# 3DHumanRehab/MOSS

Measured on AMD Instinct MI355X. Metric: train iters/sec (fwd+bwd, 512x512, ~100k Gaussians), higher is better.
Workload: dtype f32; 1 GPU; BASELINE configs[2]: 100000 Gaussians on a synthetic capsule body, 512x512, SH degree 3, step = render + L1 + 0.2(1-SSIM) + 0.5 maskL2 + backward + AdamW; one view per GPU per step; MOSS's data flow (scales + rotations + a per-Gaussian LBS transform per frame, gaussian_renderer/__init__.py:88-93) with the covariance product, the getters, the loss and AdamW as this library's kernels and the step re; target=body, input_mode=lbs, index_order=as_generated, activations=in_op, P=100000, visible=100000, num_rendered=240441, pixels=262144, parallelism=single GPU, forward=async, launch=one hipGraph replay per step, loss=full frame: L1 + 0.2 (1 - SSIM) + 0.5 mask L2 (moss_photometric_loss)

## Files before the change

moss_amd/csrc/preprocess.hip:

```cpp
#include "common.h"
#include "adamw.h"

namespace moss {

namespace {

struct M3 { float m[3][3]; };

__device__ __forceinline__ float sigmoid_act(float v) { return 1.0f / (1.0f + expf(-v)); }
__device__ __forceinline__ void activate_scale_rot(int raw, float* sc, float* q)
{
    if (raw & RAW_SCALE) { sc[0] = expf(sc[0]); sc[1] = expf(sc[1]); sc[2] = expf(sc[2]); }
    if (raw & RAW_ROTATION) {
        const float n = sqrtf(q[0] * q[0] + q[1] * q[1] + q[2] * q[2] + q[3] * q[3]);
        const float inv = 1.0f / fmaxf(n, 1e-12f);
        q[0] *= inv; q[1] *= inv; q[2] *= inv; q[3] *= inv;
    }
}
__device__ __forceinline__ void normalize_backward(const float* q, const float* y, float* g)
{
    const float n = sqrtf(q[0] * q[0] + q[1] * q[1] + q[2] * q[2] + q[3] * q[3]);
    const float inv = 1.0f / fmaxf(n, 1e-12f);
    const float yg = n >= 1e-12f ? (y[0] * g[0] + y[1] * g[1] + y[2] * g[2] + y[3] * g[3]) : 0.0f;
#pragma unroll
// ... 520 lines not shown
    for (int k = 0; k < 3; k++) dmean[k] = Rv[0][k] * dt[0] + Rv[1][k] * dt[1] + Rv[2][k] * dt[2];

    {
        const float hx = projmatrix[0] * mean.x + projmatrix[4] * mean.y + projmatrix[8] * mean.z + projmatrix[12];
        const float hy = projmatrix[1] * mean.x + projmatrix[5] * mean.y + projmatrix[9] * mean.z + projmatrix[13];
        const float hw = projmatrix[3] * mean.x + projmatrix[7] * mean.y + projmatrix[11] * mean.z + projmatrix[15];
        const float iw = 1.0f / (hw + 0.0000001f);
        const float nx = hx * iw, ny = hy * iw;
#pragma unroll
        for (int k = 0; k < 3; k++)
            dmean[k] += iw * ((projmatrix[4 * k] - nx * projmatrix[4 * k + 3]) * gmx + (projmatrix[4 * k + 1] - ny * projmatrix[4 * k + 3]) * gmy);
    }

}

__device__ __forceinline__ void scale_rot_backward(int idx, const float* dcov, const float (&A)[2][3], const float (&d2)[3],
                                                   float scale_modifier, int raw,
                                                   bool has_scales, const float (&sc_in)[3], const float (&q_in)[4],
                                                   bool has_transforms, const float (&Tm)[9], float* dscale, float* drot, float* dtf)
{
    (void)idx;
    if (has_scales) {
        float scr[3] = { sc_in[0], sc_in[1], sc_in[2] };
        float qr[4] = { q_in[0], q_in[1], q_in[2], q_in[3] };
        const float q_raw[4] = { qr[0], qr[1], qr[2], qr[3] };
        activate_scale_rot(raw, scr, qr);
        float Ap[2][3] = { { A[0][0], A[0][1], A[0][2] }, { A[1][0], A[1][1], A[1][2] } };
        float d6[6] = { dcov[0], dcov[1], dcov[2], dcov[3], dcov[4], dcov[5] };
        if (has_transforms) {
            float pre[6], d6_pre[6];
            cov3d_from_scale_rot(scr, scale_modifier, qr, pre);
            transform_cov3d_bw(Tm, pre, d6, d6_pre, dtf);
#pragma unroll
            for (int i = 0; i < 6; i++) d6[i] = d6_pre[i];
#pragma unroll
            for (int j = 0; j < 2; j++)
#pragma unroll
                for (int i = 0; i < 3; i++) Ap[j][i] = A[j][0] * Tm[i] + A[j][1] * Tm[3 + i] + A[j][2] * Tm[6 + i];
        }
        const float qw = qr[0], qx = qr[1], qy = qr[2], qz = qr[3];
        const float R[3][3] = { { 1.f - 2.f * (qy * qy + qz * qz), 2.f * (qx * qy - qw * qz), 2.f * (qx * qz + qw * qy) },
                                { 2.f * (qx * qy + qw * qz), 1.f - 2.f * (qx * qx + qz * qz), 2.f * (qy * qz - qw * qx) },
                                { 2.f * (qx * qz - qw * qy), 2.f * (qy * qz + qw * qx), 1.f - 2.f * (qx * qx + qy * qy) } };
        const float sm[3] = { scale_modifier * scr[0], scale_modifier * scr[1], scale_modifier * scr[2] };
        const float D3[3][3] = { { d6[0], 0.5f * d6[1], 0.5f * d6[2] }, { 0.5f * d6[1], d6[3], 0.5f * d6[4] }, { 0.5f * d6[2], 0.5f * d6[4], d6[5] } };
        float G[3][3];
#pragma unroll
        for (int k = 0; k < 3; k++) {
            const float u0 = Ap[0][0] * R[0][k] + Ap[0][1] * R[1][k] + Ap[0][2] * R[2][k];
            const float u1 = Ap[1][0] * R[0][k] + Ap[1][1] * R[1][k] + Ap[1][2] * R[2][k];
            const float w0 = d2[0] * u0 + d2[1] * u1, w1 = d2[1] * u0 + d2[2] * u1;
            dscale[k] = 2.0f * sm[k] * (u0 * w0 + u1 * w1);
            float col[3];
#pragma unroll
            for (int i = 0; i < 3; i++) col[i] = 2.0f * sm[k] * (D3[i][0] * R[0][k] + D3[i][1] * R[1][k] + D3[i][2] * R[2][k]);
#pragma unroll
            for (int i = 0; i < 3; i++) G[i][k] = col[i] * sm[k];
        }
        const float a0 = G[2][1] - G[1][2], a1 = G[0][2] - G[2][0], a2q = G[1][0] - G[0][1];
        const float s01 = G[0][1] + G[1][0], s02 = G[0][2] + G[2][0], s12 = G[1][2] + G[2][1];
        const float trG = G[0][0] + G[1][1] + G[2][2];
        drot[0] = 2.0f * (qx * a0 + qy * a1 + qz * a2q);
        drot[1] = 2.0f * (qy * s01 + qz * s02 + qw * a0) - 4.0f * qx * (trG - G[0][0]);
        drot[2] = 2.0f * (qx * s01 + qz * s12 + qw * a1) - 4.0f * qy * (trG - G[1][1]);
        drot[3] = 2.0f * (qx * s02 + qy * s12 + qw * a2q) - 4.0f * qz * (trG - G[2][2]);
        if (raw & RAW_SCALE) {
#pragma unroll
            for (int k = 0; k < 3; k++) dscale[k] *= scr[k];
        }
        if (raw & RAW_ROTATION) normalize_backward(q_raw, qr, drot);
    }
}

__device__ __forceinline__ uint32_t run_word_mask(uint32_t word, uint32_t c0, uint32_t c1)
{
    const uint32_t base = word << 5;
    const uint32_t lo = c0 > base ? c0 - base : 0u, hi = c1 > base ? min(c1 - base, 32u) : 0u;
    if (hi <= lo) return 0u;
    return (hi >= 32u ? 0xffffffffu : ((1u << hi) - 1u)) & ~((1u << lo) - 1u);
}
template <int NG>
__device__ __forceinline__ void coop_gather(bool is_big, uint32_t c0, uint32_t c1,
                                            const uint32_t* __restrict__ cell_valid, const float4* __restrict__ inst_grad, float* sums)
    {
        typedef float v4f __attribute__((ext_vector_type(4)));
        constexpr uint32_t OOB = 0xffffffffu, RSRC3 = 0x00020000u;
        constexpr uint32_t LPR = 64u / (uint32_t)NG;
        const __amdgpu_buffer_rsrc_t rs_msk = __builtin_amdgcn_make_buffer_rsrc((void*)cell_valid, 0, 0xffffff00u, RSRC3);
        const __amdgpu_buffer_rsrc_t rs_rec = __builtin_amdgcn_make_buffer_rsrc((void*)inst_grad, 0, 0xffffff00u, RSRC3);
        unsigned long long big = __ballot(is_big);
        const uint32_t lane = threadIdx.x & 63u, grp = lane / LPR, j = lane % LPR;
        while (big) {
            int src[NG];
#pragma unroll
            for (int g = 0; g < NG; g++) { src[g] = big ? __ffsll(big) - 1 : -1; big &= big - 1ull; }
            int my_src = src[0];
#pragma unroll
            for (int g = 1; g < NG; g++) my_src = grp == (uint32_t)g ? src[g] : my_src;
            const uint32_t bc0 = __shfl(c0, max(my_src, 0)), bc1_any = __shfl(c1, max(my_src, 0));
            const uint32_t bc1 = my_src >= 0 ? bc1_any : bc0;
            uint32_t nmax = 0u;
#pragma unroll
            for (int g = 0; g < NG; g++) {
                const uint32_t n = src[g] >= 0 ? (uint32_t)__builtin_amdgcn_readlane((int)(c1 - c0), max(src[g], 0)) : 0u;
                nmax = max(nmax, n);
            }
            float acc[9] = { 0, 0, 0, 0, 0, 0, 0, 0, 0 };
            constexpr int CPL = 8;
            for (uint32_t r0 = 0u; r0 < nmax; r0 += LPR * CPL) {
                uint32_t vw[CPL];
#pragma unroll
                for (int i = 0; i < CPL; i++) {
                    const uint32_t cell = bc0 + r0 + LPR * (uint32_t)i + j;
                    vw[i] = __builtin_amdgcn_raw_buffer_load_b32(rs_msk, cell < bc1 ? (cell >> 5) * 4u : OOB, 0, 0);
                }
                v4f ra[CPL], rb[CPL]; float rc[CPL];
#pragma unroll
                for (int i = 0; i < CPL; i++) {
                    const uint32_t cell = bc0 + r0 + LPR * (uint32_t)i + j;
                    const bool on = ((vw[i] >> (cell & 31u)) & 1u) != 0u;
                    const uint32_t o = on ? cell * (uint32_t)(GRAD_REC_FLOATS * 4) : OOB;
                    ra[i] = __builtin_amdgcn_raw_buffer_load_b128(rs_rec, o, 0, 0);
                    rb[i] = __builtin_amdgcn_raw_buffer_load_b128(rs_rec, on ? o + 16u : OOB, 0, 0);
                    rc[i] = __builtin_bit_cast(float, __builtin_amdgcn_raw_buffer_load_b32(rs_rec, on ? o + 32u : OOB, 0, 0));
                }
#pragma unroll
                for (int i = 0; i < CPL; i++) {
                    acc[0] += ra[i].x; acc[1] += ra[i].y; acc[2] += ra[i].z; acc[3] += ra[i].w;
                    acc[4] += rb[i].x; acc[5] += rb[i].y; acc[6] += rb[i].z; acc[7] += rb[i].w;
                    acc[8] += rc[i];
                }
            }
#pragma unroll
            for (int q = 0; q < 9; q++) {
#pragma unroll
                for (int d = (int)LPR / 2; d >= 1; d >>= 1) acc[q] += __shfl_xor(acc[q], d);
            }
#pragma unroll
            for (int g = 0; g < NG; g++) {
                if (src[g] >= 0) {
#pragma unroll
                    for (int q = 0; q < 9; q++) {
                        const float v = __builtin_bit_cast(float, __builtin_amdgcn_readlane(__builtin_bit_cast(int, acc[q]), g * (int)LPR));
                        if ((int)lane == src[g]) sums[q] = v;
                    }
                }
            }
        }
    }

constexpr int SH_ROW = 49;
constexpr int GATHER_CAP = 320;
constexpr int GATHER_WORDS = GATHER_CAP + 64 * 9;
template <bool STAGE_SH, bool FUSED, int LPG_L2 >
__global__ void __launch_bounds__(256) __attribute__((amdgpu_waves_per_eu(2)))
preprocess_backward_kernel(int P, int D, int M, float tan_fovx, float tan_fovy, float h_x, float h_y, float mean2d_sx, float mean2d_sy,
                           float scale_modifier,
                           const float* __restrict__ means3D, const float* __restrict__ shs,
                           const float* __restrict__ scales, const float* __restrict__ rotations,
                           const float* __restrict__ cov3D_precomp, const float* __restrict__ viewmatrix,
                           const float* __restrict__ projmatrix, const float* __restrict__ cam_pos,
                           GeomView g, const float4* __restrict__ inst_grad ,
                           const uint32_t* __restrict__ cell_valid , const uint32_t* __restrict__ header,
                           float* __restrict__ dL_dmean2D, float* __restrict__ dL_dconic, float* __restrict__ dL_dopacity,
                           float* __restrict__ dL_dcolor, float* __restrict__ dL_dmean3D, float* __restrict__ dL_dcov3D,
                           float* __restrict__ dL_dsh, float* __restrict__ dL_dscale, float* __restrict__ dL_drot,
                           const float* __restrict__ transforms, float* __restrict__ dL_dtransforms,
                           const float* __restrict__ opacities , int raw,
                           unsigned long long* __restrict__ g_stamps_dev ,
                           uint32_t* __restrict__ queues,
                           const float* __restrict__ translation , float* __restrict__ dL_dtranslation ,
                           FusedAdam fa )
{
    if (queues != nullptr && blockIdx.x == 0 && threadIdx.x < 2 * NUM_XCD_QUEUES) {
        const int line = threadIdx.x < NUM_XCD_QUEUES ? Q_BWD + (int)threadIdx.x : Q_SEG_HEAD + (int)threadIdx.x - NUM_XCD_QUEUES;
        queues[(size_t)line * QLINE_WORDS] = 0u;
    }
    float fa_bc1 = 1.0f, fa_bc2_sqrt = 1.0f;
    int fa_t = 0;
    extern __shared__ float s_sh[];
#define PSTAMP(i) if (g_stamps_dev && threadIdx.x == 0) g_stamps_dev[(size_t)blockIdx.x * 16 + (i)] = __builtin_amdgcn_s_memtime()
#define PRSTAMP(i) if (g_stamps_dev && threadIdx.x == 0) g_stamps_dev[(size_t)blockIdx.x * 16 + (i)] = __builtin_amdgcn_s_memrealtime()
    PSTAMP(0); PRSTAMP(13);
    float* const s_dsh = s_sh;
    const int gl2 = (raw >> 12) & 7;
#define rows_used ((int)blockDim.x >> LPG_L2)
    constexpr int lpg_l2 = LPG_L2;
    auto gaussian_of_row = [&](int r) -> int {
        if constexpr (LPG_L2 == 0) { return (((r >> gl2) * (int)gridDim.x + (int)blockIdx.x) << gl2) + (r & ((1 << gl2) - 1)); }
        else { return (r & ((1 << LPG_L2) - 1)) ? 0x7fffffff : (int)blockIdx.x * rows_used + (r >> LPG_L2); }
    };
    const int idx = gaussian_of_row((int)threadIdx.x);
    const bool in_range = idx < P;
    const int idc = min(idx, P - 1);
    constexpr int SH_J = LPG_L2 == 0 ? 12 : 1;
    typedef float v4f_sh __attribute__((ext_vector_type(4)));
    constexpr uint32_t SH_OOB = 0xffffffffu;
    const int na_D = (3 * (D + 1) * (D + 1) + 3) >> 2;
    const __amdgpu_buffer_rsrc_t rs_shs = __builtin_amdgcn_make_buffer_rsrc((void*)shs, 0, 0xffffff00u, 0x00020000u);
    v4f_sh shv[12];
    if (STAGE_SH) {
        const size_t total4 = (size_t)P * 12;
#pragma unroll
        for (int j = 0; j < SH_J; j++) {
            const int f = (int)threadIdx.x + j * (int)blockDim.x;
            size_t a;
            if constexpr (LPG_L2 == 0) a = min((size_t)gaussian_of_row(f / 12) * 12 + (size_t)(f % 12), total4 - 1);
            else a = f / 12 < rows_used ? min((size_t)min(gaussian_of_row((f / 12) << lpg_l2), P - 1) * 12 + (size_t)(f % 12), total4 - 1) : total4 - 1;
            shv[j] = __builtin_amdgcn_raw_buffer_load_b128(rs_shs, (f % 12) < na_D ? (uint32_t)a * 16u : SH_OOB, 0, 0);
        }
    }
    const uint32_t tt_raw = g.tiles_touched[idc], off_raw = g.rec_offsets[idc] + g.group_rbase[idc >> 8], cells_raw = g.rec_count[idc], hdr_flags = header[2];
    float in_x[3], in_T[9] = { 0.f, 0.f, 0.f, 0.f, 0.f, 0.f, 0.f, 0.f, 0.f }, in_t[3] = { 0.f, 0.f, 0.f }, in_c6[6], in_sc[3] = { 0.f, 0.f, 0.f }, in_q[4] = { 0.f, 0.f, 0.f, 0.f };
    float in_opa = 0.f;
#pragma unroll
    for (int i = 0; i < 3; i++) in_x[i] = means3D[3 * (size_t)idc + i];
    if (transforms != nullptr) {
#pragma unroll
        for (int i = 0; i < 9; i++) in_T[i] = transforms[9 * (size_t)idc + i];
    }
    if ((raw & RAW_POSE) && translation != nullptr) {
#pragma unroll
        for (int i = 0; i < 3; i++) in_t[i] = translation[3 * (size_t)idc + i];
    }
    {
        const float* c6p = (cov3D_precomp != nullptr) ? cov3D_precomp + 6 * (size_t)idc : g.cov3D + 6 * (size_t)idc;
#pragma unroll
        for (int i = 0; i < 6; i++) in_c6[i] = c6p[i];
    }
    if (scales != nullptr) {
#pragma unroll
        for (int i = 0; i < 3; i++) in_sc[i] = scales[3 * (size_t)idc + i];
#pragma unroll
        for (int i = 0; i < 4; i++) in_q[i] = rotations[4 * (size_t)idc + i];
    }
    if (raw & RAW_OPACITY) in_opa = opacities[idc];
    const uint8_t in_clamped = g.clamped[idc];
    if (STAGE_SH) {
#pragma unroll
        for (int j = 0; j < SH_J; j++) {
            const int f = threadIdx.x + j * blockDim.x;
            if (LPG_L2 == 0 || f / 12 < rows_used) {
                float* d = &s_sh[((f / 12) << lpg_l2) * SH_ROW + (f % 12) * 4];
                d[0] = shv[j].x; d[1] = shv[j].y; d[2] = shv[j].z; d[3] = shv[j].w;
            }
        }
    }
    const uint32_t n_inst = in_range ? tt_raw : 0u;
#pragma unroll
    for (int i = 0; i < 3; i++) { asm volatile("" : "+v"(in_x[i])); asm volatile("" : "+v"(in_t[i])); asm volatile("" : "+v"(in_sc[i])); }
#pragma unroll
    for (int i = 0; i < 9; i++) asm volatile("" : "+v"(in_T[i]));
#pragma unroll
    for (int i = 0; i < 6; i++) asm volatile("" : "+v"(in_c6[i]));
#pragma unroll
    for (int i = 0; i < 4; i++) asm volatile("" : "+v"(in_q[i]));
    asm volatile("" : "+v"(in_opa));
    float3 gcol = make_float3(0, 0, 0); float gmx = 0, gmy = 0, gca = 0, gcb = 0, gcc = 0, gop = 0;
    float dmean[3] = { 0, 0, 0 }, dcov[6] = { 0, 0, 0, 0, 0, 0 }, dscale[3] = { 0, 0, 0 }, drot[4] = { 0, 0, 0, 0 };
    float dtf[9] = { 0, 0, 0, 0, 0, 0, 0, 0, 0 }, dpose_t[3] = { 0, 0, 0 };
    float A_cov[2][3] = { { 0, 0, 0 }, { 0, 0, 0 } }, d2_cov[3] = { 0, 0, 0 };
    const bool visible = n_inst > 0 && !(hdr_flags & (ERRFLAG_OVERFLOW | ERRFLAG_FORWARD_ONLY));
    const bool fa_on = FUSED && !(hdr_flags & (ERRFLAG_OVERFLOW | ERRFLAG_FORWARD_ONLY));

    constexpr uint32_t COOP_WORDS = 16, MID_CELLS = 96;
    const uint32_t c0 = visible ? off_raw : 0u, c1 = c0 + (visible ? cells_raw : 0u);
    const uint32_t word0 = c0 >> 5, n_words = c1 > c0 ? ((c1 + 31u) >> 5) - word0 : 0u;
    const bool mid_size = LPG_L2 == 0 && (c1 - c0) > MID_CELLS && n_words <= COOP_WORDS;
    {
        const bool mine = n_words != 0u && n_words <= COOP_WORDS && !mid_size;
        PSTAMP(8);
        const int lane_g = (int)(threadIdx.x & 63u);
        uint32_t g_c0 = c0, g_c1 = c1, g_n = mine ? n_words : 0u;
        if constexpr (LPG_L2 == 4) {
            g_c0 = (uint32_t)__shfl((int)g_c0, lane_g & ~15); g_c1 = (uint32_t)__shfl((int)g_c1, lane_g & ~15); g_n = (uint32_t)__shfl((int)g_n, lane_g & ~15);
        }
        const bool has_word = (uint32_t)(lane_g & 15) < g_n;
        uint32_t wmax = LPG_L2 == 4 ? (has_word ? 1u : 0u) : (mine ? n_words : 0u);
#pragma unroll
        for (int d = 32; d >= 1; d >>= 1) wmax = max(wmax, (uint32_t)__shfl_xor((int)wmax, d));
        typedef float v4f __attribute__((ext_vector_type(4)));
        constexpr uint32_t OOB = 0xffffffffu, RSRC3 = 0x00020000u;
        const __amdgpu_buffer_rsrc_t rs_msk = __builtin_amdgcn_make_buffer_rsrc((void*)cell_valid, 0, 0xffffff00u, RSRC3);
        const __amdgpu_buffer_rsrc_t rs_rec = __builtin_amdgcn_make_buffer_rsrc((void*)inst_grad, 0, 0xffffff00u, RSRC3);
        uint32_t pp[COOP_WORDS], mm[COOP_WORDS];
#pragma unroll
        for (int k = 0; k < (int)COOP_WORDS; k++) pp[k] = LPG_L2 == 4 ? (k == 0 ? (g_c0 >> 5) + (uint32_t)(lane_g & 15) : 0u) : word0 + (uint32_t)k;
        PSTAMP(9);
#pragma unroll
        for (int k = 0; k < (int)COOP_WORDS; k++) {
            if constexpr (LPG_L2 == 4) mm[k] = k == 0 ? (__builtin_amdgcn_raw_buffer_load_b32(rs_msk, has_word ? pp[0] * 4u : OOB, 0, 0) & run_word_mask(pp[0], g_c0, g_c1)) : 0u;
            else mm[k] = __builtin_amdgcn_raw_buffer_load_b32(rs_msk, (mine && (uint32_t)k < n_words) ? pp[k] * 4u : OOB, 0, 0) & run_word_mask(pp[k], c0, c1);
        }
        PSTAMP(10);
        uint32_t cnt = 0u;
#pragma unroll
        for (int k = 0; k < (int)COOP_WORDS; k++) cnt += (uint32_t)__popc(mm[k]);
        uint32_t incl = cnt;
        uint32_t bmax = 0u;
#pragma unroll
        for (int k = 0; k < (int)COOP_WORDS; k++) {
            const uint32_t pc = (uint32_t)__popc(mm[k]), sh = 8u * (uint32_t)(k >> 2);
            bmax = max(bmax & (0xffu << sh), pc << sh) | (bmax & ~(0xffu << sh));
        }
        {
            const int lane_ = (int)(threadIdx.x & 63u);
#pragma unroll
            for (int d = 1; d < 64; d <<= 1) { const uint32_t y = (uint32_t)__shfl_up((int)incl, d); if (lane_ >= d) incl += y; }
#pragma unroll
            for (int d = 32; d >= 1; d >>= 1) {
                const uint32_t o = (uint32_t)__shfl_xor((int)bmax, d);
                uint32_t r = 0u;
#pragma unroll
                for (int b = 0; b < 4; b++) r |= max(bmax & (0xffu << (8 * b)), o & (0xffu << (8 * b)));
                bmax = r;
            }
        }
        const uint32_t W_all = (uint32_t)__shfl((int)incl, 63);
        const uint32_t passes = (W_all + (uint32_t)GATHER_CAP - 1u) / (uint32_t)GATHER_CAP;
        const uint32_t direct_trips = ((bmax & 0xffu) + 1u) / 2u + (((bmax >> 8) & 0xffu) + 1u) / 2u + (((bmax >> 16) & 0xffu) + 1u) / 2u + ((bmax >> 24) + 1u) / 2u;
        const bool balanced = LPG_L2 == 4 ? true :
                              __builtin_amdgcn_readfirstlane((int)(passes == 1u ? direct_trips >= 5u : passes * 8u < direct_trips)) != 0;
        if (!balanced) {
#pragma unroll
        for (int kb = 0; kb < (int)COOP_WORDS; kb += 4) {
            if ((uint32_t)kb < wmax) {
                uint32_t bits[4] = { mm[kb], mm[kb + 1], mm[kb + 2], mm[kb + 3] };
                do {
                    v4f rr[4][2][3];
#pragma unroll
                    for (int k = 0; k < 4; k++) {
#pragma unroll
                        for (int j = 0; j < 2; j++) {
                            const bool any = bits[k] != 0u;
                            const uint32_t sl = any ? (uint32_t)(__ffs((int)bits[k]) - 1) : 0u;
                            bits[k] &= bits[k] - 1u;
                            const uint32_t o = any ? ((pp[kb + k] << 5) + sl) * (uint32_t)(GRAD_REC_FLOATS * 4) : OOB;
// ... 13 lines not shown
                    }
                } while (__ballot((bits[0] | bits[1] | bits[2] | bits[3]) != 0u) != 0ull);
            }
        }
        } else
        {
            uint32_t* const w_desc = reinterpret_cast<uint32_t*>(s_sh + (STAGE_SH ? blockDim.x * SH_ROW : 0)) + (threadIdx.x >> 6) * GATHER_WORDS;
            float* const w_row = reinterpret_cast<float*>(w_desc + GATHER_CAP);
            const int lane = (int)(threadIdx.x & 63u);
            const uint32_t base = incl - cnt, W = W_all;
            uint32_t run_base = base, run_cnt = cnt;
            bool head_ok = true;
            if constexpr (LPG_L2 == 4) {
                const uint32_t gbase = (uint32_t)__shfl((int)base, lane & ~15), gend = (uint32_t)__shfl((int)incl, lane | 15);
                head_ok = base == gbase;
                run_base = gbase; run_cnt = (lane & 15) == 0 ? gend - gbase : 0u;
            }
            for (uint32_t w0 = 0u; w0 < W; w0 += (uint32_t)GATHER_CAP) {
                const uint32_t w1 = min(W, w0 + (uint32_t)GATHER_CAP);
                __builtin_amdgcn_wave_barrier();
                {
                    uint32_t j = base;
#pragma unroll
                    for (int k = 0; k < (int)COOP_WORDS; k++) {
                        if ((uint32_t)k < wmax) {
                            uint32_t bits = mm[k];
                            while (__ballot(bits != 0u) != 0ull) {
                                if (bits != 0u) {
                                    const uint32_t sl = (uint32_t)(__ffs((int)bits) - 1);
                                    bits &= bits - 1u;
                                    if (j >= w0 && j < w1) w_desc[j - w0] = ((j == base && head_ok) ? 0x80000000u : 0u) | ((pp[k] << 5) + sl);
                                    j++;
                                }
                            }
                        }
                    }
                }
                __builtin_amdgcn_wave_barrier();
                constexpr int ROWS = GATHER_CAP / 64;
                const int nrows = (int)((w1 - w0 + 63u) / 64u);
                v4f ra[ROWS], rb[ROWS]; float rc[ROWS]; uint32_t dsc[ROWS];
#pragma unroll
                for (int r = 0; r < ROWS; r++) {
                    const uint32_t w = w0 + 64u * (uint32_t)r + (uint32_t)lane;
                    const bool on = w < w1;
                    dsc[r] = on ? w_desc[w - w0] : 0x80000000u;
                    const uint32_t o = on ? (dsc[r] & 0x7fffffffu) * (uint32_t)(GRAD_REC_FLOATS * 4) : OOB;
                    ra[r] = __builtin_amdgcn_raw_buffer_load_b128(rs_rec, o, 0, 0);
                    rb[r] = __builtin_amdgcn_raw_buffer_load_b128(rs_rec, on ? o + 16u : OOB, 0, 0);
                    rc[r] = __builtin_bit_cast(float, __builtin_amdgcn_raw_buffer_load_b32(rs_rec, on ? o + 32u : OOB, 0, 0));
                }
#pragma unroll
                for (int r = 0; r < ROWS; r++) {
                    if (r < nrows) {
                        float v[9] = { ra[r].x, ra[r].y, ra[r].z, ra[r].w, rb[r].x, rb[r].y, rb[r].z, rb[r].w, rc[r] };
                        uint32_t f = (dsc[r] >> 31) | (lane == 0 ? 1u : 0u);
#pragma unroll
                        for (int d = 1; d < 64; d <<= 1) {
                            const uint32_t fu = (uint32_t)__shfl_up((int)f, d);
                            float t[9];
#pragma unroll
                            for (int q = 0; q < 9; q++) t[q] = __shfl_up(v[q], d);
                            const bool take = lane >= d && f == 0u;
#pragma unroll
                            for (int q = 0; q < 9; q++) v[q] += take ? t[q] : 0.0f;
                            f |= lane >= d ? fu : 0u;
                        }
                        __builtin_amdgcn_wave_barrier();
#pragma unroll
                        for (int q = 0; q < 9; q++) w_row[lane * 9 + q] = v[q];
                        __builtin_amdgcn_wave_barrier();
                        const uint32_t row0 = w0 + 64u * (uint32_t)r, row1 = min(w1, row0 + 64u);
                        const uint32_t lo = max(run_base, row0), hi = min(run_base + run_cnt, row1);
                        if (lo < hi) {
                            const float* e = w_row + (hi - 1u - row0) * 9u;
                            gcol.x += e[0]; gcol.y += e[1]; gcol.z += e[2]; gmx += e[3];
                            gmy += e[4]; gca += e[5]; gcb += e[6]; gcc += e[7]; gop += e[8];
                        }
                    }
                }
            }
        }
        PSTAMP(11);
    }
    {
        float sums[9] = { gcol.x, gcol.y, gcol.z, gmx, gmy, gca, gcb, gcc, gop };
        if constexpr (LPG_L2 == 0) coop_gather<4>(mid_size, c0, c1, cell_valid, inst_grad, sums);
        coop_gather<1>(n_words > COOP_WORDS, c0, c1, cell_valid, inst_grad, sums);
        gcol.x = sums[0]; gcol.y = sums[1]; gcol.z = sums[2]; gmx = sums[3]; gmy = sums[4]; gca = sums[5]; gcb = sums[6]; gcc = sums[7]; gop = sums[8];
    }
    PSTAMP(12);
    PSTAMP(1);
    if (STAGE_SH) __syncthreads();
    PSTAMP(2);
    gmx *= mean2d_sx; gmy *= mean2d_sy; gca *= -0.5f; gcb *= -0.5f; gcc *= -0.5f;
    if (FUSED) {
        const int t_prev = reinterpret_cast<const int*>(fa.step_state)[0], lr_flag = reinterpret_cast<const int*>(fa.step_state)[ADAMW_LR_VALID_WORD];
        fa_t = adamw_step_begin(fa.step_state, fa.betas, false, fa_bc1, fa_bc2_sqrt, t_prev);
        if (lr_flag != 0) {
#pragma unroll
            for (int i = 0; i < 5; i++) if (fa.lr_segment[i] >= 0) fa.lr[i] = fa.step_state[ADAMW_LR_WORD0 + fa.lr_segment[i]];
            if (fa.lr_segment[1] >= 0) fa.lr_sh_rest = fa.step_state[ADAMW_LR2_WORD0 + fa.lr_segment[1]];
        }
    }
    if (fa_on && blockIdx.x == 0 && threadIdx.x == 0) adamw_cache_next(fa.step_state, fa.betas, fa_t);
    const bool fa_scalars = fa_on && in_range && (fa.tensors & (OPT_MEANS | OPT_OPACITY | OPT_SCALES | OPT_ROTATIONS));
    float fa_p[11], fa_m[11], fa_v[11];
#pragma unroll
    for (int i = 0; i < 11; i++) { fa_p[i] = 0.f; fa_m[i] = 0.f; fa_v[i] = 0.f; }
    if (fa_scalars) {
        const size_t i3 = 3 * (size_t)idx;
        if (fa.tensors & OPT_MEANS) {
#pragma unroll
            for (int i = 0; i < 3; i++) { fa_p[i] = fa.p[0][i3 + i]; fa_m[i] = fa.m[0][i3 + i]; fa_v[i] = fa.v[0][i3 + i]; }
        }
        if (fa.tensors & OPT_OPACITY) { fa_p[3] = fa.p[2][idx]; fa_m[3] = fa.m[2][idx]; fa_v[3] = fa.v[2][idx]; }
        if (fa.tensors & OPT_SCALES) {
#pragma unroll
            for (int i = 0; i < 3; i++) { fa_p[4 + i] = fa.p[3][i3 + i]; fa_m[4 + i] = fa.m[3][i3 + i]; fa_v[4 + i] = fa.v[3][i3 + i]; }
        }
        if (fa.tensors & OPT_ROTATIONS) {
            const float4 a = reinterpret_cast<const float4*>(fa.p[4])[idx], b = reinterpret_cast<const float4*>(fa.m[4])[idx], c = reinterpret_cast<const float4*>(fa.v[4])[idx];
            fa_p[7] = a.x; fa_p[8] = a.y; fa_p[9] = a.z; fa_p[10] = a.w; fa_m[7] = b.x; fa_m[8] = b.y; fa_m[9] = b.z; fa_m[10] = b.w;
            fa_v[7] = c.x; fa_v[8] = c.y; fa_v[9] = c.z; fa_v[10] = c.w;
        }
    }
    constexpr int FA_HOIST = SH_J < 10 ? SH_J : 10;
    float4 fa_m4[12], fa_v4[12];
    const bool fa_sh = STAGE_SH && fa_on && (fa.tensors & OPT_SH);
    const __amdgpu_buffer_rsrc_t rs_fm = __builtin_amdgcn_make_buffer_rsrc((void*)fa.m[1], 0, 0xffffff00u, 0x00020000u);
    const __amdgpu_buffer_rsrc_t rs_fv = __builtin_amdgcn_make_buffer_rsrc((void*)fa.v[1], 0, 0xffffff00u, 0x00020000u);
    if (fa_sh) {
#pragma unroll
        for (int j = 0; j < FA_HOIST; j++) {
            const int f = (int)threadIdx.x + j * (int)blockDim.x;
            const size_t a = (size_t)min(gaussian_of_row(LPG_L2 == 0 ? f / 12 : (min(f / 12, rows_used - 1) << lpg_l2)), P - 1) * 12 + (size_t)(f % 12);
            const uint32_t o = (f % 12) < fa.sh_active_parts ? (uint32_t)a * 16u : SH_OOB;
            const v4f_sh mq = __builtin_amdgcn_raw_buffer_load_b128(rs_fm, o, 0, 0), vq = __builtin_amdgcn_raw_buffer_load_b128(rs_fv, o, 0, 0);
            fa_m4[j] = make_float4(mq.x, mq.y, mq.z, mq.w); fa_v4[j] = make_float4(vq.x, vq.y, vq.z, vq.w);
        }
    }
    if (in_range) {
    dL_dmean2D[3 * (size_t)idx] = gmx; dL_dmean2D[3 * (size_t)idx + 1] = gmy; dL_dmean2D[3 * (size_t)idx + 2] = 0.0f;
    if (dL_dconic != nullptr) reinterpret_cast<float4*>(dL_dconic)[idx] = make_float4(gca, gcb, 0.0f, gcc);
    if (raw & RAW_OPACITY) {
        const float sg = sigmoid_act(in_opa);
        gop = gop * ((1.0f - sg) * sg);
    }
    if (dL_dopacity != nullptr) dL_dopacity[idx] = gop;
    if (dL_dcolor != nullptr) { dL_dcolor[3 * (size_t)idx] = gcol.x; dL_dcolor[3 * (size_t)idx + 1] = gcol.y; dL_dcolor[3 * (size_t)idx + 2] = gcol.z; }

    float* dsh = STAGE_SH ? &s_dsh[threadIdx.x * SH_ROW]
                          : ((M > 0 && dL_dsh != nullptr) ? dL_dsh + (size_t)idx * M * 3 : nullptr);

    if (visible) {
        const float3 xc = make_float3(in_x[0], in_x[1], in_x[2]);
        float3 mean = xc;
        if (raw & RAW_POSE) mean = pose_point(in_T, xc, make_float3(in_t[0], in_t[1], in_t[2]));
        cov_proj_backward(idx, gca, gcb, gcc, gmx, gmy, tan_fovx, tan_fovy, h_x, h_y, in_c6, viewmatrix, projmatrix, mean, dmean, dcov, A_cov, d2_cov);

        PSTAMP(3);
        if (shs != nullptr) {
            const float* sh = STAGE_SH ? &s_sh[threadIdx.x * SH_ROW] : shs + (size_t)idx * M * 3;
            const float vx = mean.x - cam_pos[0], vy = mean.y - cam_pos[1], vz = mean.z - cam_pos[2];
            const float vlen = sqrtf(vx * vx + vy * vy + vz * vz);
            const float x = vx / vlen, y = vy / vlen, z = vz / vlen;
            const uint8_t cl = in_clamped;
            const float gc[3] = { (cl & 1) ? 0.0f : gcol.x, (cl & 2) ? 0.0f : gcol.y, (cl & 4) ? 0.0f : gcol.z };
            float basis[16], gbx[16], gby[16], gbz[16];
            const int used = (D + 1) * (D + 1);
            basis[0] = SH_C0; gbx[0] = 0.f; gby[0] = 0.f; gbz[0] = 0.f;
            if (D > 0) {
                basis[1] = -SH_C1 * y; gbx[1] = 0.f;    gby[1] = -SH_C1; gbz[1] = 0.f;
                basis[2] = SH_C1 * z;  gbx[2] = 0.f;    gby[2] = 0.f;    gbz[2] = SH_C1;
                basis[3] = -SH_C1 * x; gbx[3] = -SH_C1; gby[3] = 0.f;    gbz[3] = 0.f;
            }
            if (D > 1) {
                const float xx = x * x, yy = y * y, zz = z * z;
                basis[4] = SH_C2[0] * (x * y);            gbx[4] = SH_C2[0] * y;          gby[4] = SH_C2[0] * x;          gbz[4] = 0.f;
                basis[5] = SH_C2[1] * (y * z);            gbx[5] = 0.f;                   gby[5] = SH_C2[1] * z;          gbz[5] = SH_C2[1] * y;
                basis[6] = SH_C2[2] * (2.f * zz - xx - yy); gbx[6] = SH_C2[2] * (-2.f * x); gby[6] = SH_C2[2] * (-2.f * y); gbz[6] = SH_C2[2] * (4.f * z);
                basis[7] = SH_C2[3] * (x * z);            gbx[7] = SH_C2[3] * z;          gby[7] = 0.f;                   gbz[7] = SH_C2[3] * x;
                basis[8] = SH_C2[4] * (xx - yy);          gbx[8] = SH_C2[4] * (2.f * x);  gby[8] = SH_C2[4] * (-2.f * y); gbz[8] = 0.f;
                if (D > 2) {
                    const float xy = x * y, yz = y * z, xz = x * z;
                    basis[9] = SH_C3[0] * (y * (3.f * xx - yy));            gbx[9] = SH_C3[0] * (6.f * xy);              gby[9] = SH_C3[0] * (3.f * (xx - yy));           gbz[9] = 0.f;
                    basis[10] = SH_C3[1] * (xy * z);                        gbx[10] = SH_C3[1] * yz;                     gby[10] = SH_C3[1] * xz;                          gbz[10] = SH_C3[1] * xy;
                    basis[11] = SH_C3[2] * (y * (4.f * zz - xx - yy));      gbx[11] = SH_C3[2] * (-2.f * xy);            gby[11] = SH_C3[2] * (4.f * zz - xx - 3.f * yy);   gbz[11] = SH_C3[2] * (8.f * yz);
                    basis[12] = SH_C3[3] * (z * (2.f * zz - 3.f * xx - 3.f * yy)); gbx[12] = SH_C3[3] * (-6.f * xz);     gby[12] = SH_C3[3] * (-6.f * yz);                 gbz[12] = SH_C3[3] * (6.f * zz - 3.f * xx - 3.f * yy);
                    basis[13] = SH_C3[4] * (x * (4.f * zz - xx - yy));      gbx[13] = SH_C3[4] * (4.f * zz - 3.f * xx - yy); gby[13] = SH_C3[4] * (-2.f * xy);             gbz[13] = SH_C3[4] * (8.f * xz);
                    basis[14] = SH_C3[5] * (z * (xx - yy));                 gbx[14] = SH_C3[5] * (2.f * xz);             gby[14] = SH_C3[5] * (-2.f * yz);                 gbz[14] = SH_C3[5] * (xx - yy);
                    basis[15] = SH_C3[6] * (x * (xx - 3.f * yy));           gbx[15] = SH_C3[6] * (3.f * (xx - yy));      gby[15] = SH_C3[6] * (-6.f * xy);                 gbz[15] = 0.f;
                }
            }
            float ddx = 0.f, ddy = 0.f, ddz = 0.f;
#pragma unroll
            for (int k = 0; k < 16; k++) {
                if (k < used) {
                    const float sk = sh[3 * k] * gc[0] + sh[3 * k + 1] * gc[1] + sh[3 * k + 2] * gc[2];
                    dsh[3 * k] = basis[k] * gc[0]; dsh[3 * k + 1] = basis[k] * gc[1]; dsh[3 * k + 2] = basis[k] * gc[2];
                    ddx += gbx[k] * sk; ddy += gby[k] * sk; ddz += gbz[k] * sk;
                }
            }
            for (int k = used; k < M; k++) { dsh[3 * k] = 0.0f; dsh[3 * k + 1] = 0.0f; dsh[3 * k + 2] = 0.0f; }
            const float nd = x * ddx + y * ddy + z * ddz, il = 1.0f / vlen;
            dmean[0] += (ddx - x * nd) * il; dmean[1] += (ddy - y * nd) * il; dmean[2] += (ddz - z * nd) * il;
        }


        PSTAMP(4);
        scale_rot_backward(idx, dcov, A_cov, d2_cov, scale_modifier, raw, scales != nullptr, in_sc, in_q, transforms != nullptr, in_T, dscale, drot, dtf);
        if (raw & RAW_POSE) {
            const float gp[3] = { dmean[0], dmean[1], dmean[2] }, xv[3] = { xc.x, xc.y, xc.z };
            const float (&Tm)[9] = in_T;
#pragma unroll
            for (int a = 0; a < 3; a++)
#pragma unroll
                for (int c = 0; c < 3; c++) dtf[3 * a + c] += gp[a] * xv[c];
#pragma unroll
            for (int c = 0; c < 3; c++) dmean[c] = Tm[c] * gp[0] + Tm[3 + c] * gp[1] + Tm[6 + c] * gp[2];
            dpose_t[0] = gp[0]; dpose_t[1] = gp[1]; dpose_t[2] = gp[2];
        }
    } else if (dsh != nullptr) {
        for (int k = 0; k < 3 * M; k++) dsh[k] = 0.0f;
    }
    if (visible && dsh != nullptr && shs == nullptr) {
        for (int k = 0; k < 3 * M; k++) dsh[k] = 0.0f;
    }

    if (dL_dmean3D != nullptr) {
#pragma unroll
        for (int i = 0; i < 3; i++) dL_dmean3D[3 * (size_t)idx + i] = dmean[i];
    }
    if (dL_dcov3D != nullptr) {
#pragma unroll
        for (int i = 0; i < 6; i++) dL_dcov3D[6 * (size_t)idx + i] = dcov[i];
    }
    if (dL_dscale != nullptr) {
#pragma unroll
        for (int i = 0; i < 3; i++) dL_dscale[3 * (size_t)idx + i] = dscale[i];
    }
    if (dL_drot != nullptr) reinterpret_cast<float4*>(dL_drot)[idx] = make_float4(drot[0], drot[1], drot[2], drot[3]);
    if (dL_dtransforms != nullptr) {
#pragma unroll
        for (int i = 0; i < 9; i++) dL_dtransforms[9 * (size_t)idx + i] = dtf[i];
    }
    if (dL_dtranslation != nullptr) {
#pragma unroll
        for (int i = 0; i < 3; i++) dL_dtranslation[3 * (size_t)idx + i] = dpose_t[i];
    }
    if (fa_scalars) {
        const float ib1 = 1.0f / fa_bc1, ib2 = 1.0f / fa_bc2_sqrt;
        const size_t i3 = 3 * (size_t)idx;
        const float gv[11] = { dmean[0], dmean[1], dmean[2], gop, dscale[0], dscale[1], dscale[2], drot[0], drot[1], drot[2], drot[3] };
#pragma unroll
        for (int i = 0; i < 11; i++) {
            const float lr = i < 3 ? fa.lr[0] : i == 3 ? fa.lr[2] : i < 7 ? fa.lr[3] : fa.lr[4];
            adamw_element(fa_p[i], gv[i], fa_m[i], fa_v[i], lr, fa.betas, fa.eps, fa.weight_decay, ib1, ib2);
        }
        if (fa.tensors & OPT_MEANS) {
#pragma unroll
            for (int i = 0; i < 3; i++) { fa.p[0][i3 + i] = fa_p[i]; fa.m[0][i3 + i] = fa_m[i]; fa.v[0][i3 + i] = fa_v[i]; }
        }
        if (fa.tensors & OPT_OPACITY) { fa.p[2][idx] = fa_p[3]; fa.m[2][idx] = fa_m[3]; fa.v[2][idx] = fa_v[3]; }
        if (fa.tensors & OPT_SCALES) {
#pragma unroll
            for (int i = 0; i < 3; i++) { fa.p[3][i3 + i] = fa_p[4 + i]; fa.m[3][i3 + i] = fa_m[4 + i]; fa.v[3][i3 + i] = fa_v[4 + i]; }
        }
        if (fa.tensors & OPT_ROTATIONS) {
            reinterpret_cast<float4*>(fa.p[4])[idx] = make_float4(fa_p[7], fa_p[8], fa_p[9], fa_p[10]);
            reinterpret_cast<float4*>(fa.m[4])[idx] = make_float4(fa_m[7], fa_m[8], fa_m[9], fa_m[10]);
            reinterpret_cast<float4*>(fa.v[4])[idx] = make_float4(fa_v[7], fa_v[8], fa_v[9], fa_v[10]);
        }
    }
    }
    PSTAMP(5);
    if (STAGE_SH) {
        __syncthreads();
        if (dL_dsh != nullptr) {
            float4* dst = reinterpret_cast<float4*>(dL_dsh);
            const int n_write = (raw & SH_GRAD_ACTIVE_ONLY) ? na_D : 12;
            for (int f = threadIdx.x; f < (LPG_L2 == 0 ? (int)blockDim.x : rows_used) * 12; f += blockDim.x) {
                const int gi = gaussian_of_row((f / 12) << lpg_l2);
                if (gi < P && (f % 12) < n_write) {
                    const float* r = &s_dsh[((f / 12) << lpg_l2) * SH_ROW + (f % 12) * 4];
                    dst[(size_t)gi * 12 + (size_t)(f % 12)] = make_float4(r[0], r[1], r[2], r[3]);
                }
            }
        }
        if (fa_on && (fa.tensors & OPT_SH)) {
            const float ib1 = 1.0f / fa_bc1, ib2 = 1.0f / fa_bc2_sqrt;
            float4* const pw = reinterpret_cast<float4*>(fa.p[1]);
            float4* const mw = reinterpret_cast<float4*>(fa.m[1]);
            float4* const vw = reinterpret_cast<float4*>(fa.v[1]);
            float4 p4[12];
            float4 (&m4)[12] = fa_m4, (&v4)[12] = fa_v4;
            const __amdgpu_buffer_rsrc_t rs_fp = __builtin_amdgcn_make_buffer_rsrc((void*)fa.p[1], 0, 0xffffff00u, 0x00020000u);
            const int n_act = fa.sh_active_parts;
            const bool skip_rest = fa.sh_inactive_zero != 0;
#pragma unroll
            for (int j = 0; j < SH_J; j++) {
                const int f = (int)threadIdx.x + j * (int)blockDim.x, part = f % 12;
                const size_t a = (size_t)min(gaussian_of_row(LPG_L2 == 0 ? f / 12 : (min(f / 12, rows_used - 1) << lpg_l2)), P - 1) * 12 + (size_t)part;
                const uint32_t o = (uint32_t)a * 16u;
                const v4f_sh pq = __builtin_amdgcn_raw_buffer_load_b128(rs_fp, (part < n_act || !skip_rest) ? o : SH_OOB, 0, 0);
                p4[j] = make_float4(pq.x, pq.y, pq.z, pq.w);
                if (j >= FA_HOIST) {
                    const v4f_sh mq = __builtin_amdgcn_raw_buffer_load_b128(rs_fm, part < n_act ? o : SH_OOB, 0, 0);
                    const v4f_sh vq = __builtin_amdgcn_raw_buffer_load_b128(rs_fv, part < n_act ? o : SH_OOB, 0, 0);
                    m4[j] = make_float4(mq.x, mq.y, mq.z, mq.w); v4[j] = make_float4(vq.x, vq.y, vq.z, vq.w);
                }
            }
#pragma unroll
            for (int j = 0; j < SH_J; j++) {
                const int f = (int)threadIdx.x + j * (int)blockDim.x, part = f % 12;
                const int q = LPG_L2 == 0 ? f / 12 : min(f / 12, rows_used - 1);
                const int gi = (LPG_L2 == 0 || f / 12 < rows_used) ? gaussian_of_row(q << lpg_l2) : 0x7fffffff;
                const float* r = &s_dsh[(q << lpg_l2) * SH_ROW + part * 4];
                float pe[4] = { p4[j].x, p4[j].y, p4[j].z, p4[j].w }, me[4] = { m4[j].x, m4[j].y, m4[j].z, m4[j].w };
                float ve[4] = { v4[j].x, v4[j].y, v4[j].z, v4[j].w };
                if (part < n_act) {
#pragma unroll
                    for (int k = 0; k < 4; k++)
                        adamw_element(pe[k], r[k], me[k], ve[k], (part == 0 && k < 3) ? fa.lr[1] : fa.lr_sh_rest, fa.betas, fa.eps,
                                      fa.weight_decay, ib1, ib2);
                    if (gi < P) {
                        const size_t a = (size_t)gi * 12 + (size_t)part;
                        pw[a] = make_float4(pe[0], pe[1], pe[2], pe[3]);
                        mw[a] = make_float4(me[0], me[1], me[2], me[3]);
                        vw[a] = make_float4(ve[0], ve[1], ve[2], ve[3]);
                    }
                } else if (!skip_rest) {
                    float pn[4];
#pragma unroll
                    for (int k = 0; k < 4; k++) pn[k] = __fmul_rn(pe[k], __fsub_rn(1.0f, __fmul_rn(fa.lr_sh_rest, fa.weight_decay)));
                    if (gi < P && (pn[0] != pe[0] || pn[1] != pe[1] || pn[2] != pe[2] || pn[3] != pe[3]))
                        pw[(size_t)gi * 12 + (size_t)part] = make_float4(pn[0], pn[1], pn[2], pn[3]);
                }
            }
        }
    }
    if (fa_on && threadIdx.x == 0) adamw_step_end(fa.step_state, fa_t);
    PSTAMP(6); PRSTAMP(14);
#undef PSTAMP
#undef PRSTAMP
#undef rows_used
}

__global__ void __launch_bounds__(256)
mark_visible_kernel(int P, const float* __restrict__ means3D, const float* __restrict__ viewmatrix, uint8_t* __restrict__ present)
{
    const int idx = blockIdx.x * blockDim.x + threadIdx.x;
    if (idx >= P) return;
    float view[16];
#pragma unroll
    for (int i = 0; i < 16; i++) view[i] = viewmatrix[i];
    const float3 p = make_float3(means3D[3 * (size_t)idx], means3D[3 * (size_t)idx + 1], means3D[3 * (size_t)idx + 2]);
    const float3 pv = xform4x3(p, view);
    present[idx] = (pv.z <= 0.2f) ? 0 : 1;
}

__global__ void __launch_bounds__(256)
export_geometry_kernel(int P, GeomView g, float* depths, float* means2D, float* conic_opacity, float* rgb,
                       uint32_t* tiles_touched, uint8_t* clamped, float* cov3D)
{
    const int idx = blockIdx.x * blockDim.x + threadIdx.x;
    if (idx >= P) return;
    const bool vis = g.tiles_touched[idx] > 0;
    const float4 z4 = make_float4(0, 0, 0, 0);
    const float4 a = vis ? g.geo[4 * (size_t)idx] : z4, b = vis ? g.geo[4 * (size_t)idx + 1] : z4, c = vis ? g.geo[4 * (size_t)idx + 2] : z4;
    if (depths) depths[idx] = c.w;
    if (means2D) { means2D[2 * (size_t)idx] = a.x; means2D[2 * (size_t)idx + 1] = a.y; }
    if (conic_opacity) reinterpret_cast<float4*>(conic_opacity)[idx] = b;
    if (rgb) { rgb[3 * (size_t)idx] = c.x; rgb[3 * (size_t)idx + 1] = c.y; rgb[3 * (size_t)idx + 2] = c.z; }
    if (tiles_touched) tiles_touched[idx] = g.tiles_touched[idx];
    if (clamped) {
        const uint8_t cl = vis ? g.clamped[idx] : 0;
        clamped[3 * (size_t)idx] = cl & 1; clamped[3 * (size_t)idx + 1] = (cl >> 1) & 1; clamped[3 * (size_t)idx + 2] = (cl >> 2) & 1;
    }
    if (cov3D) for (int i = 0; i < 6; i++) cov3D[6 * (size_t)idx + i] = g.cov3D[6 * (size_t)idx + i];
}

}

void launch_preprocess_forward(const FrameParams& fp, const float* means3D, const float* shs, const float* colors_precomp,
                               const float* opacities, const float* scales, const float* rotations, const float* cov3D_precomp,
                               const float* transforms, const float* translation, GeomView g, ImageView im, int* radii_out, hipStream_t s,
                               uint64_t* scatter_keys, uint32_t key_stride)
{
    const int T = fp.gx * fp.gy;
    const int lds_hist = (T <= MAX_LDS_TILES) ? 1 : 0;
    if (!lds_hist) scatter_keys = nullptr;
    static const int per_thread = knob("MOSS_PREPROCESS_ITEMS", 1);
    int blocks = (fp.P + 256 * per_thread - 1) / (256 * per_thread);
    if (blocks < 1) blocks = 1;
    const size_t lds_h = lds_hist ? (size_t)((T + 3) & ~3) * sizeof(uint32_t) : 0, lds_s = (size_t)256 * SH_ROW_F * sizeof(float);
    static const bool big_lds = hipFuncSetAttribute(reinterpret_cast<const void*>(preprocess_forward_kernel), hipFuncAttributeMaxDynamicSharedMemorySize, 80 * 1024) == hipSuccess;
    const int stage_sh = (fp.M == 16 && shs != nullptr && colors_precomp == nullptr && (reinterpret_cast<uintptr_t>(shs) & 15u) == 0 &&
                          (size_t)fp.P * 192u < 0xffffff00u  &&
                          lds_h + lds_s <= (big_lds ? 80u * 1024u : 65536u) && knob("MOSS_PREFWD_STAGE", 1)) ? 1 : 0;
    const size_t lds = lds_h + (stage_sh ? lds_s : 0);
    MOSS_LAUNCH_TIMED(preprocess_forward_kernel, dim3(blocks), dim3(256), lds, s,
                       fp.P, fp.D, fp.M, fp.W, fp.H, fp.gx, fp.gy, fp.tan_fovx, fp.tan_fovy, fp.focal_x, fp.focal_y,
                       fp.scale_modifier, fp.prefiltered, means3D, shs, colors_precomp, opacities, scales, rotations,
                       cov3D_precomp, fp.view_dev, fp.proj_dev, fp.campos_dev, g, im.tile_count, im.flags_acc, radii_out, lds_hist, stage_sh,
                       transforms, fp.raw,
                       (g_stamps && knob("MOSS_SORT_STAMPS", 0)) ? g_stamps + 131072 + 32768 : nullptr, translation, scatter_keys, key_stride);
}

static int prebwd_resident_per_cu(int threads)
{
    static const int occ = [&] {
        const size_t lds_bytes_staged = (size_t)threads * SH_ROW * sizeof(float) + (size_t)((threads + 63) / 64) * GATHER_WORDS * 4;
        int o = 0;
        if (hipOccupancyMaxActiveBlocksPerMultiprocessor(&o, preprocess_backward_kernel<true, true, 4>, threads, lds_bytes_staged) != hipSuccess || o < 1) o = 1;
        return o;
    }();
    return occ;
}

void launch_preprocess_backward(const FrameParams& fp, const float* means3D, const float* shs, const float* colors_precomp,
                                const float* opacities, const float* scales, const float* rotations, const float* cov3D_precomp,
                                GeomView g, BinView b, const uint32_t* header, uint32_t* queues,
                                float* dL_dmean2D, float* dL_dconic, float* dL_dopacity, float* dL_dcolor, float* dL_dmean3D,
                                float* dL_dcov3D, float* dL_dsh, float* dL_dscale, float* dL_drot,
                                const float* transforms, float* dL_dtransforms, const float* translation, float* dL_dtranslation, hipStream_t s,
                                const FusedAdam* fused)
{
    (void)colors_precomp;
    const FusedAdam fa = fused ? *fused : FusedAdam();
    static const int threads = std::max(64, knob("MOSS_PREBWD_THREADS", 64) & ~63);
    static const int gl2_env = knob("MOSS_PREBWD_GROUP_LOG2", 0);
    const bool stage = fp.M == 16 && shs != nullptr && (dL_dsh != nullptr || (fa.tensors & OPT_SH)) && (size_t)fp.P * 192u < 0xffffff00u &&
                       (knob("MOSS_PREBWD_STAGE", 1) || (fa.tensors & OPT_SH)) &&
                       (reinterpret_cast<uintptr_t>(shs) & 15u) == 0 && (reinterpret_cast<uintptr_t>(dL_dsh) & 15u) == 0;
    static const int lpg_env = knob("MOSS_PREBWD_LPG_LOG2", -1);
    int lpg_l2 = 0;
    if (stage) {
        const long long resident = (long long)prebwd_resident_per_cu(threads) * device_cus();
        if (((long long)fp.P + (threads >> 4) - 1) / (threads >> 4) <= resident) lpg_l2 = 4;
        if (lpg_env >= 0) lpg_l2 = lpg_env >= 4 ? 4 : 0;
    }
    const int blocks = (fp.P + (threads >> lpg_l2) - 1) / (threads >> lpg_l2);
    const int resident_per_cu = prebwd_resident_per_cu(threads);
    const int gl2 = gl2_env ? std::max(4, std::min(6, gl2_env))
                            : (((fp.raw & HINT_SPATIAL_ORDER) && blocks <= resident_per_cu * device_cus()) ? 4 : 6);
#define LAUNCH_PB(STAGE, FUSE, LPG)                                                                                             \
    MOSS_LAUNCH_TIMED((preprocess_backward_kernel<STAGE, FUSE, LPG>), dim3(blocks), dim3(threads),                             \
                       ((STAGE) ? (size_t)threads * SH_ROW * sizeof(float) : 0) + (size_t)((threads + 63) / 64) * GATHER_WORDS * 4, s,                                               \
                       fp.P, fp.D, fp.M, fp.tan_fovx, fp.tan_fovy, fp.focal_x, fp.focal_y, -0.5f * (float)fp.W, -0.5f * (float)fp.H, fp.scale_modifier, \
                       means3D, shs, scales, rotations, cov3D_precomp, fp.view_dev, fp.proj_dev, fp.campos_dev,                 \
                       g, b.inst_grad, b.cell_valid, header, dL_dmean2D, dL_dconic, \
                       dL_dopacity, dL_dcolor, dL_dmean3D, dL_dcov3D, dL_dsh, dL_dscale, dL_drot, transforms, dL_dtransforms, opacities, fp.raw | (gl2 << 12), g_stamps, queues, translation, dL_dtranslation, fa)
    if (stage && lpg_l2 == 4) { if (fa.tensors != 0u) LAUNCH_PB(true, true, 4); else LAUNCH_PB(true, false, 4); }
    else if (fa.tensors != 0u) { if (stage) LAUNCH_PB(true, true, 0); else LAUNCH_PB(false, true, 0); }
    else if (stage) LAUNCH_PB(true, false, 0); else LAUNCH_PB(false, false, 0);
#undef LAUNCH_PB
}

void launch_mark_visible(int P, const float* means3D, const float* view16_dev, uint8_t* present, hipStream_t s)
{
    hipLaunchKernelGGL(mark_visible_kernel, dim3((P + 255) / 256), dim3(256), 0, s, P, means3D, view16_dev, present);
}

void launch_export_geometry(int P, GeomView g, float* depths, float* means2D, float* conic_opacity, float* rgb,
                            uint32_t* tiles_touched, uint8_t* clamped, float* cov3D, hipStream_t s)
{
    hipLaunchKernelGGL(export_geometry_kernel, dim3((P + 255) / 256), dim3(256), 0, s, P, g, depths, means2D, conic_opacity, rgb,
                       tiles_touched, clamped, cov3D);
}

}
```

Baseline: 5500 iters/s.

## Store SH gradient factors instead of full dSH rows in fused preprocess backward

In the fused staged-SH path, each thread now writes 19 factors (16 SH basis values plus 3 clamped color gradients) into a separate LDS area instead of the full 48-float dSH row. The SH gradient is rebuilt from these factors when writing dL_dsh and inside the fused AdamW update. The AdamW step also takes parameter values for active parts from the already staged LDS SH copy, so it only loads them from global memory for parts above the active degree. This cuts LDS writes and global parameter reads, but the LDS layout is resized and the launch size and occupancy query now go through a new helper function.

Result: no change. 5539 iters/s (median of 6 runs) (+0.7%).

```diff
diff --git a/moss_amd/csrc/preprocess.hip b/moss_amd/csrc/preprocess.hip
--- a/moss_amd/csrc/preprocess.hip
+++ b/moss_amd/csrc/preprocess.hip
@@ -696,6 +696,14 @@
 constexpr int SH_ROW = 49;
 constexpr int GATHER_CAP = 320;
 constexpr int GATHER_WORDS = GATHER_CAP + 64 * 9;
+constexpr int FAC_ROW = 21;
+static_assert(64 * FAC_ROW >= GATHER_WORDS, "the factor rows of a wave cover its gather area");
+constexpr size_t prebwd_lds_bytes(int threads, bool stage, bool fused)
+{
+    return (stage ? (size_t)threads * SH_ROW * sizeof(float) : 0) +
+           ((stage && fused) ? (size_t)threads * FAC_ROW * sizeof(float) : (size_t)((threads + 63) / 64) * GATHER_WORDS * 4);
+}
+static_assert(prebwd_lds_bytes(64, true, true) <= 20 * 1024, "the fused per-Gaussian backward: at most 20 KB of LDS per 64-thread block");
 template <bool STAGE_SH, bool FUSED, int LPG_L2 >
 __global__ void __launch_bounds__(256) __attribute__((amdgpu_waves_per_eu(2)))
 preprocess_backward_kernel(int P, int D, int M, float tan_fovx, float tan_fovy, float h_x, float h_y, float mean2d_sx, float mean2d_sy,
@@ -727,6 +735,8 @@
 #define PRSTAMP(i) if (g_stamps_dev && threadIdx.x == 0) g_stamps_dev[(size_t)blockIdx.x * 16 + (i)] = __builtin_amdgcn_s_memrealtime()
     PSTAMP(0); PRSTAMP(13);
     float* const s_dsh = s_sh;
+    constexpr bool FACTORS = STAGE_SH && FUSED;
+#define s_fac (s_sh + blockDim.x * SH_ROW)
     const int gl2 = (raw >> 12) & 7;
 #define rows_used ((int)blockDim.x >> LPG_L2)
     constexpr int lpg_l2 = LPG_L2;
@@ -1046,6 +1056,7 @@
 
     float* dsh = STAGE_SH ? &s_dsh[threadIdx.x * SH_ROW]
                           : ((M > 0 && dL_dsh != nullptr) ? dL_dsh + (size_t)idx * M * 3 : nullptr);
+    float* const fac = FACTORS ? &s_fac[threadIdx.x * FAC_ROW] : nullptr;
 
     if (visible) {
         const float3 xc = make_float3(in_x[0], in_x[1], in_x[2]);
@@ -1088,15 +1099,20 @@
                 }
             }
             float ddx = 0.f, ddy = 0.f, ddz = 0.f;
+            if constexpr (FACTORS) {
+#pragma unroll
+                for (int k = 0; k < 16; k++) fac[k] = k < used ? basis[k] : 0.0f;
+                fac[16] = gc[0]; fac[17] = gc[1]; fac[18] = gc[2];
+            }
 #pragma unroll
             for (int k = 0; k < 16; k++) {
                 if (k < used) {
                     const float sk = sh[3 * k] * gc[0] + sh[3 * k + 1] * gc[1] + sh[3 * k + 2] * gc[2];
-                    dsh[3 * k] = basis[k] * gc[0]; dsh[3 * k + 1] = basis[k] * gc[1]; dsh[3 * k + 2] = basis[k] * gc[2];
+                    if constexpr (!FACTORS) { dsh[3 * k] = basis[k] * gc[0]; dsh[3 * k + 1] = basis[k] * gc[1]; dsh[3 * k + 2] = basis[k] * gc[2]; }
                     ddx += gbx[k] * sk; ddy += gby[k] * sk; ddz += gbz[k] * sk;
                 }
             }
-            for (int k = used; k < M; k++) { dsh[3 * k] = 0.0f; dsh[3 * k + 1] = 0.0f; dsh[3 * k + 2] = 0.0f; }
+            if constexpr (!FACTORS) for (int k = used; k < M; k++) { dsh[3 * k] = 0.0f; dsh[3 * k + 1] = 0.0f; dsh[3 * k + 2] = 0.0f; }
             const float nd = x * ddx + y * ddy + z * ddz, il = 1.0f / vlen;
             dmean[0] += (ddx - x * nd) * il; dmean[1] += (ddy - y * nd) * il; dmean[2] += (ddz - z * nd) * il;
         }
@@ -1115,10 +1131,17 @@
             for (int c = 0; c < 3; c++) dmean[c] = Tm[c] * gp[0] + Tm[3 + c] * gp[1] + Tm[6 + c] * gp[2];
             dpose_t[0] = gp[0]; dpose_t[1] = gp[1]; dpose_t[2] = gp[2];
         }
+    } else if constexpr (FACTORS) {
+#pragma unroll
+        for (int k = 0; k < 19; k++) fac[k] = 0.0f;
     } else if (dsh != nullptr) {
         for (int k = 0; k < 3 * M; k++) dsh[k] = 0.0f;
     }
     if (visible && dsh != nullptr && shs == nullptr) {
+        if constexpr (FACTORS) {
+#pragma unroll
+            for (int k = 0; k < 19; k++) fac[k] = 0.0f;
+        } else
         for (int k = 0; k < 3 * M; k++) dsh[k] = 0.0f;
     }
 
@@ -1171,6 +1194,31 @@
     PSTAMP(5);
     if (STAGE_SH) {
         __syncthreads();
+        auto sh_factor_grads = [&](int row, int part, float (&gq)[4]) {
+            const float* fr = &s_fac[row * FAC_ROW];
+            const int r0 = part % 3, b0 = (4 * part) / 3, i_end = 3 * (D + 1) * (D + 1);
+            const float ba = fr[b0], bb = fr[b0 + 1], ca = fr[16], cb = fr[17], cc = fr[18];
+#pragma unroll
+            for (int e = 0; e < 4; e++) {
+                const int t = r0 + e, tc = t < 3 ? t : t - 3;
+                const float gv = __fmul_rn(t < 3 ? ba : bb, tc == 0 ? ca : tc == 1 ? cb : cc);
+                gq[e] = 4 * part + e < i_end ? gv : 0.0f;
+            }
+        };
+        if constexpr (FACTORS) {
+            if (dL_dsh != nullptr) {
+                float4* dst = reinterpret_cast<float4*>(dL_dsh);
+                const int n_write = (raw & SH_GRAD_ACTIVE_ONLY) ? na_D : 12;
+                for (int f = threadIdx.x; f < (LPG_L2 == 0 ? (int)blockDim.x : rows_used) * 12; f += blockDim.x) {
+                    const int gi = gaussian_of_row((f / 12) << lpg_l2);
+                    if (gi < P && (f % 12) < n_write) {
+                        float gq[4];
+                        sh_factor_grads((f / 12) << lpg_l2, f % 12, gq);
+                        dst[(size_t)gi * 12 + (size_t)(f % 12)] = make_float4(gq[0], gq[1], gq[2], gq[3]);
+                    }
+                }
+            }
+        } else
         if (dL_dsh != nullptr) {
             float4* dst = reinterpret_cast<float4*>(dL_dsh);
             const int n_write = (raw & SH_GRAD_ACTIVE_ONLY) ? na_D : 12;
@@ -1182,7 +1230,7 @@
                 }
             }
         }
-        if (fa_on && (fa.tensors & OPT_SH)) {
+        if constexpr (FACTORS) if (fa_on && (fa.tensors & OPT_SH)) {
             const float ib1 = 1.0f / fa_bc1, ib2 = 1.0f / fa_bc2_sqrt;
             float4* const pw = reinterpret_cast<float4*>(fa.p[1]);
             float4* const mw = reinterpret_cast<float4*>(fa.m[1]);
@@ -1192,27 +1240,43 @@
             const __amdgpu_buffer_rsrc_t rs_fp = __builtin_amdgcn_make_buffer_rsrc((void*)fa.p[1], 0, 0xffffff00u, 0x00020000u);
             const int n_act = fa.sh_active_parts;
             const bool skip_rest = fa.sh_inactive_zero != 0;
+            const bool p_above = na_D < 12 && (n_act > na_D || !skip_rest);
 #pragma unroll
             for (int j = 0; j < SH_J; j++) {
                 const int f = (int)threadIdx.x + j * (int)blockDim.x, part = f % 12;
                 const size_t a = (size_t)min(gaussian_of_row(LPG_L2 == 0 ? f / 12 : (min(f / 12, rows_used - 1) << lpg_l2)), P - 1) * 12 + (size_t)part;
                 const uint32_t o = (uint32_t)a * 16u;
-                const v4f_sh pq = __builtin_amdgcn_raw_buffer_load_b128(rs_fp, (part < n_act || !skip_rest) ? o : SH_OOB, 0, 0);
-                p4[j] = make_float4(pq.x, pq.y, pq.z, pq.w);
                 if (j >= FA_HOIST) {
                     const v4f_sh mq = __builtin_amdgcn_raw_buffer_load_b128(rs_fm, part < n_act ? o : SH_OOB, 0, 0);
                     const v4f_sh vq = __builtin_amdgcn_raw_buffer_load_b128(rs_fv, part < n_act ? o : SH_OOB, 0, 0);
                     m4[j] = make_float4(mq.x, mq.y, mq.z, mq.w); v4[j] = make_float4(vq.x, vq.y, vq.z, vq.w);
                 }
+                p4[j] = make_float4(0.f, 0.f, 0.f, 0.f);
+            }
+            if (p_above) {
+#pragma unroll
+                for (int j = 0; j < SH_J; j++) {
+                    const int f = (int)threadIdx.x + j * (int)blockDim.x, part = f % 12;
+                    const size_t a = (size_t)min(gaussian_of_row(LPG_L2 == 0 ? f / 12 : (min(f / 12, rows_used - 1) << lpg_l2)), P - 1) * 12 + (size_t)part;
+                    const v4f_sh pq = __builtin_amdgcn_raw_buffer_load_b128(rs_fp, (part >= na_D && (part < n_act || !skip_rest)) ? (uint32_t)a * 16u : SH_OOB, 0, 0);
+                    p4[j] = make_float4(pq.x, pq.y, pq.z, pq.w);
+                }
             }
 #pragma unroll
             for (int j = 0; j < SH_J; j++) {
                 const int f = (int)threadIdx.x + j * (int)blockDim.x, part = f % 12;
                 const int q = LPG_L2 == 0 ? f / 12 : min(f / 12, rows_used - 1);
                 const int gi = (LPG_L2 == 0 || f / 12 < rows_used) ? gaussian_of_row(q << lpg_l2) : 0x7fffffff;
-                const float* r = &s_dsh[(q << lpg_l2) * SH_ROW + part * 4];
-                float pe[4] = { p4[j].x, p4[j].y, p4[j].z, p4[j].w }, me[4] = { m4[j].x, m4[j].y, m4[j].z, m4[j].w };
+                const float* ps = &s_sh[(q << lpg_l2) * SH_ROW + part * 4];
+                float r[4];
+                sh_factor_grads(q << lpg_l2, part, r);
+                float pe[4], me[4] = { m4[j].x, m4[j].y, m4[j].z, m4[j].w };
                 float ve[4] = { v4[j].x, v4[j].y, v4[j].z, v4[j].w };
+                {
+                    const float pa[4] = { p4[j].x, p4[j].y, p4[j].z, p4[j].w };
+#pragma unroll
+                    for (int k = 0; k < 4; k++) pe[k] = part < na_D ? ps[k] : pa[k];
+                }
                 if (part < n_act) {
 #pragma unroll
                     for (int k = 0; k < 4; k++)
@@ -1239,6 +1303,7 @@
 #undef PSTAMP
 #undef PRSTAMP
 #undef rows_used
+#undef s_fac
 }
 
 __global__ void __launch_bounds__(256)
@@ -1305,7 +1370,7 @@
 static int prebwd_resident_per_cu(int threads)
 {
     static const int occ = [&] {
-        const size_t lds_bytes_staged = (size_t)threads * SH_ROW * sizeof(float) + (size_t)((threads + 63) / 64) * GATHER_WORDS * 4;
+        const size_t lds_bytes_staged = prebwd_lds_bytes(threads, true, true);
         int o = 0;
         if (hipOccupancyMaxActiveBlocksPerMultiprocessor(&o, preprocess_backward_kernel<true, true, 4>, threads, lds_bytes_staged) != hipSuccess || o < 1) o = 1;
         return o;
@@ -1341,7 +1406,7 @@
                             : (((fp.raw & HINT_SPATIAL_ORDER) && blocks <= resident_per_cu * device_cus()) ? 4 : 6);
 #define LAUNCH_PB(STAGE, FUSE, LPG)                                                                                             \
     MOSS_LAUNCH_TIMED((preprocess_backward_kernel<STAGE, FUSE, LPG>), dim3(blocks), dim3(threads),                             \
-                       ((STAGE) ? (size_t)threads * SH_ROW * sizeof(float) : 0) + (size_t)((threads + 63) / 64) * GATHER_WORDS * 4, s,                                               \
+                       prebwd_lds_bytes(threads, STAGE, FUSE), s,                                                                 \
                        fp.P, fp.D, fp.M, fp.tan_fovx, fp.tan_fovy, fp.focal_x, fp.focal_y, -0.5f * (float)fp.W, -0.5f * (float)fp.H, fp.scale_modifier, \
                        means3D, shs, scales, rotations, cov3D_precomp, fp.view_dev, fp.proj_dev, fp.campos_dev,                 \
                        g, b.inst_grad, b.cell_valid, header, dL_dmean2D, dL_dconic, \
```
